# tachitachi/SR-WaveNet

Measured on NVIDIA B200. Metric: audio samples/sec, higher is better.
Workload: dtype f16

## Files before the change

sr-wavenet_b200/csrc/fused.cu:

```cuda
#include "common.cuh"
#include "mol.cuh"
#include "umma.cuh"
#include "philox.cuh"
#include <cuda_fp16.h>
#include <algorithm>
#include <cstdlib>

namespace fused {

constexpr int kTile = 128;
__host__ __device__ constexpr int tiles_of(bool teacher) { return teacher ? 3 : 4; }
__host__ __device__ constexpr int chunk_of(bool teacher) { return kTile * tiles_of(teacher); }
constexpr int kHalo = 512;
constexpr int kMaxLayers = 40;
constexpr int kMaxSeg = 8;

constexpr int kWfBytes = 64 * 32 * 2;
constexpr int kWrsTeacher = 32 * 160 * 2;
constexpr int kWrsStudent = 32 * 32 * 2;
constexpr int kH1Bytes = 128 * 128 * 2;
constexpr int kH2Bytes = 128 * 32 * 2;

struct Seg { int b, t_start, t_out, t_end; };

struct Params {
  const uint8_t* packed;
  const float* x_in;
  const float* x_scored;
  const float* cb;
  uint8_t* rings;
  const Seg* segs;
  const int* nseg;
  uint32_t* flags;
  int G;
  long long wait_limit;
  NoiseSpec noise;
  float* logits_out;
  float* nll_out;
  double* nll_partial;
  float* scale_out;
  float* mean_out;
  float* x_out;
  int* err;
#ifdef SRWN_TUNING
  long long* trace;
  int trace_chunk;
#endif
  int T, L, P, frames, O, M;
  int ring_bytes_per_team;
  int dil[kMaxLayers];
  int ring_off[kMaxLayers];
  int rsuf[kMaxLayers + 1];
};

template <bool TEACHER>
struct SmemMapT {
  static constexpr int NT = tiles_of(TEACHER);
  static constexpr int rows = kHalo + NT * kTile;
  static constexpr int hbuf = 0;
  static constexpr int hbuf_bytes = 4 * rows * 16;
  static constexpr int cbuf = hbuf + 2 * hbuf_bytes;
  static constexpr int cbuf_bytes = 4 * kTile * 16;
  static constexpr int wst = cbuf + NT * cbuf_bytes;
  static constexpr int wst_bytes = kWfBytes + (TEACHER ? kWrsTeacher : kWrsStudent);
  static constexpr int head = wst + 2 * wst_bytes;
  static constexpr int bias = head + (TEACHER ? kH1Bytes + kH2Bytes : 0);
  static constexpr int hbias = bias + kMaxLayers * 32 * 4;
  static constexpr int front = hbias + (128 + 128 + 32 + 64 + 4) * 4;
  static constexpr int cbs = front + 64 * 4;
  static constexpr int bars = cbs + NT * (kMaxLayers + 1) * 32 * 4;
  static constexpr int n_bars = 40;
  static constexpr int misc = bars + n_bars * 8;
  static constexpr int total = misc + 64;
};
static_assert(SmemMapT<true>::total <= 232448 && SmemMapT<false>::total <= 232448, "shared memory budget");
static_assert(3 * 16 * kTile * 16 <= 2 * SmemMapT<true>::hbuf_bytes, "head operand overlay");

template <int NT>
struct BarT {
  static constexpr int D1 = 0;
  static constexpr int D2 = NT;
  static constexpr int HD = 2 * NT;
  static constexpr int WFULL = 4 * NT;
  static constexpr int WEMPTY = WFULL + 2;
  static constexpr int HALO = WFULL + 4;
  static constexpr int G1 = WFULL + 6;
  static constexpr int HDD = WFULL + 8;
  static constexpr int TAIL = HDD + NT;
  static constexpr int C2 = TAIL + 1;
  static constexpr int count = C2 + 2 * NT;
};
static_assert(BarT<3>::count <= 40 && BarT<4>::count <= 40, "barrier slots");

using namespace umma;

__device__ __forceinline__ uint32_t gate2(f2_t a) {
  float a0, a1;
  upk(a, a0, a1);
  const f2_t f = pk(tanh_fast(a0), tanh_fast(a1));
  const f2_t s = mul2(f, f);
  f2_t t = fma2(s, pk(0.0017294071149080992f, 0.0017294071149080992f), pk(-0.020638039335608482f, -0.020638039335608482f));
  t = fma2(s, t, pk(0.2499687224626541f, 0.2499687224626541f));
  const f2_t c = fma2(f, pk(0.5f, 0.5f), mul2(s, t));
  float c0, c1;
  upk(c, c0, c1);
  return pack2(c0, c1);
}

__device__ __forceinline__ void store_row(uint8_t* buf, int rows_per_kc, int row, const float* v) {
#pragma unroll
  for (int kc = 0; kc < 4; kc++) {
    uint4 q;
    q.x = pack2(v[kc * 8 + 0], v[kc * 8 + 1]); q.y = pack2(v[kc * 8 + 2], v[kc * 8 + 3]);
    q.z = pack2(v[kc * 8 + 4], v[kc * 8 + 5]); q.w = pack2(v[kc * 8 + 6], v[kc * 8 + 7]);
    *reinterpret_cast<uint4*>(buf + ((size_t)kc * rows_per_kc + row) * 16) = q;
  }
}
__device__ __forceinline__ void store_row_packed(uint8_t* buf, int rows_per_kc, int row, const uint32_t* w) {
#pragma unroll
  for (int kc = 0; kc < 4; kc++)
    *reinterpret_cast<uint4*>(buf + ((size_t)kc * rows_per_kc + row) * 16) =
        make_uint4(w[kc * 4 + 0], w[kc * 4 + 1], w[kc * 4 + 2], w[kc * 4 + 3]);
}

#ifndef SRWN_TUNING
#define TRACE(role, layer, slot) do {} while (0)
#else
#define TRACE(role, layer, slot)                                                            \
  do {                                                                                      \
    if (tracing) p.trace[((role) * kMaxLayers + (layer)) * 12 + (slot)] = clock64();      \
  } while (0)
#endif

constexpr int kLoadWarp = 0;
__host__ __device__ constexpr int threads_of(bool handoff, int nt) { return (1 + 4 * nt + (handoff ? 1 : 0)) * 32; }

__device__ __noinline__ bool flag_spin(const uint32_t* f, uint32_t need, volatile int* abort_flag, const int* gerr, int code, long long limit) {
  const long long t0 = clock64();
  int spins = 0;
  uint32_t v;
  while (true) {
    __nanosleep(32);
    asm volatile("ld.acquire.gpu.global.u32 %0, [%1];" : "=r"(v) : "l"(f) : "memory");
    if (v >= need) return true;
    if (*abort_flag) return false;
    if (((++spins) & 1023) == 0 && *reinterpret_cast<const volatile int*>(gerr)) return false;
    if (clock64() - t0 > limit) {
      if (atomicCAS((int*)abort_flag, 0, 1) == 0) ((int*)abort_flag)[1] = code;
      return false;
    }
  }
}
__device__ __forceinline__ bool flag_try(const uint32_t* f, uint32_t need) {
  uint32_t v;
  asm volatile("ld.acquire.gpu.global.u32 %0, [%1];" : "=r"(v) : "l"(f) : "memory");
  if (v < need) return false;
  asm volatile("fence.proxy.async;" ::: "memory");
  return true;
}
__device__ __forceinline__ bool flag_wait(const uint32_t* f, uint32_t need, volatile int* abort_flag, const int* gerr, int code, long long limit) {
  uint32_t v;
  asm volatile("ld.acquire.gpu.global.u32 %0, [%1];" : "=r"(v) : "l"(f) : "memory");
  if (v < need && !flag_spin(f, need, abort_flag, gerr, code, limit)) return false;
  asm volatile("fence.proxy.async;" ::: "memory");
  return true;
}
__device__ __forceinline__ void ring_rows_done(uint32_t counter_addr, uint32_t rows) {
  asm volatile("red.release.cta.shared::cta.add.u32 [%0], %1;" ::"r"(counter_addr), "r"(rows) : "memory");
}
__device__ __forceinline__ int ring_rows_of(int d, int m, int chunk) {
  const int lo = max(chunk - d, m * kTile), hi = (m + 1) * kTile;
  return hi > lo ? hi - lo : 0;
}
__device__ __forceinline__ uint32_t ld_acquire_cta_shared(uint32_t addr) {
  uint32_t v;
  asm volatile("ld.acquire.cta.shared::cta.u32 %0, [%1];" : "=r"(v) : "r"(addr) : "memory");
  return v;
}
__device__ __forceinline__ void flag_publish(uint32_t* f, uint32_t chunks) {
  asm volatile("red.release.gpu.global.max.u32 [%0], %1;" ::"l"(f), "r"(chunks) : "memory");
}

template <bool TEACHER, bool HANDOFF>
__global__ void __launch_bounds__(threads_of(HANDOFF, tiles_of(TEACHER)), 1) k_fused(const Params p) {
  constexpr int NT = tiles_of(TEACHER), CH = NT * kTile;
  constexpr int kThreads = threads_of(HANDOFF, NT);
  constexpr int kPubWarp = 1 + 4 * NT;
  constexpr int TCOLS = TEACHER ? 160 : 64;
  using SM = SmemMapT<TEACHER>;
  constexpr int ROWS = SM::rows;
  using BR = BarT<NT>;
  constexpr int BAR_D1 = BR::D1, BAR_D2 = BR::D2, BAR_HD = BR::HD, BAR_WFULL = BR::WFULL, BAR_WEMPTY = BR::WEMPTY, BAR_HALO = BR::HALO,
                BAR_G1 = BR::G1, BAR_HDD = BR::HDD, BAR_TAIL = BR::TAIL, BAR_C2 = BR::C2;
  (void)BAR_HDD; (void)BAR_C2; (void)kPubWarp;
  extern __shared__ __align__(1024) uint8_t smem[];
  const int tid = threadIdx.x, lane = tid & 31, warp = tid >> 5;
  const uint32_t sbase = smem_u32(smem);
  volatile int* abort_flag = reinterpret_cast<volatile int*>(smem + SM::misc + 8);
  uint32_t* tmem_slot = reinterpret_cast<uint32_t*>(smem + SM::misc);
  auto bar = [&](int i) { return sbase + SM::bars + i * 8; };
  const int L = p.L;
  constexpr int wrs_bytes = TEACHER ? kWrsTeacher : kWrsStudent;
  constexpr int layer_bytes = kWfBytes + wrs_bytes;
  constexpr int wrs_rows = TEACHER ? 160 : 32;

  if (tid == 0) {
    for (int i = 0; i < NT; i++) {
      mbar_init(bar(BAR_D1 + i), 1); mbar_init(bar(BAR_D2 + i), 1); mbar_init(bar(BAR_HDD + i), 1);
      mbar_init(bar(BAR_C2 + 2 * i), 1); mbar_init(bar(BAR_C2 + 2 * i + 1), 1);
      mbar_init(bar(BAR_HD + 2 * i), kTile); mbar_init(bar(BAR_HD + 2 * i + 1), kTile);
    }
    for (int i = 0; i < 2; i++) {
      mbar_init(bar(BAR_WFULL + i), 1); mbar_init(bar(BAR_WEMPTY + i), NT);
      mbar_init(bar(BAR_HALO + i), 1); mbar_init(bar(BAR_G1 + i), NT);
    }
    mbar_init(bar(BAR_TAIL), 1);
    abort_flag[0] = 0; abort_flag[1] = 0;
    for (int i = 0; i < NT; i++) reinterpret_cast<volatile uint32_t*>(smem + SM::misc + 16)[i] = 0;
    asm volatile("fence.mbarrier_init.release.cluster;" ::: "memory");
  }
  {
    const uint8_t* pk_ = p.packed;
    const size_t off_fixed = (size_t)L * layer_bytes;
    const float* fbias = reinterpret_cast<const float*>(pk_ + off_fixed);
    float* s_bias = reinterpret_cast<float*>(smem + SM::bias);
    for (int i = tid; i < L * 32; i += kThreads) s_bias[i] = fbias[i];
    const float* ffront = fbias + kMaxLayers * 32;
    float* s_front = reinterpret_cast<float*>(smem + SM::front);
    for (int i = tid; i < 64; i += kThreads) s_front[i] = ffront[i];
    const float* fhb = ffront + 64;
    float* s_hb = reinterpret_cast<float*>(smem + SM::hbias);
    for (int i = tid; i < 128 + 128 + 32 + 64 + 4; i += kThreads) s_hb[i] = fhb[i];
    if (TEACHER) {
      const uint4* src = reinterpret_cast<const uint4*>(reinterpret_cast<const uint8_t*>(fhb + 128 + 128 + 32 + 64 + 4));
      uint4* dst = reinterpret_cast<uint4*>(smem + SM::head);
      for (int i = tid; i < (kH1Bytes + kH2Bytes) / 16; i += kThreads) dst[i] = src[i];
    }
  }
  fence_async_smem();
  if (warp == kLoadWarp) {
    asm volatile("tcgen05.alloc.cta_group::1.sync.aligned.shared::cta.b32 [%0], %1;" ::"r"(smem_u32(tmem_slot)), "r"(512));
    asm volatile("tcgen05.relinquish_alloc_permit.cta_group::1.sync.aligned;" ::);
  }
  tc_fence_before();
  __syncthreads();
  tc_fence_after();
  const uint32_t tmem = *tmem_slot;

  const int G = p.G, team = (int)blockIdx.x / G, member = (int)blockIdx.x % G;
  const Seg* segs = p.segs + (size_t)team * kMaxSeg;
  const int nseg = p.nseg[team];
  uint8_t* ring = p.rings + (size_t)team * p.ring_bytes_per_team;
  uint32_t* flags = p.flags + (size_t)team * kMaxLayers;
  const uint32_t ringcnt = sbase + SM::misc + 16;
  uint32_t pub_expect = 0;
  int seq = 0;
  int u0e = 0, u0o = 0, lay_base = 0;
  int chunk_idx = 0;
  int head_idx = 0;
  int tail_idx = 0;
  double nll_acc = 0.0;
  const bool elected = elect_one();

  for (int si = 0; si < nseg; si++) {
    const Seg sg = segs[si];
    for (int t0 = sg.t_start; t0 < sg.t_end; t0 += CH) {
      const int n = seq++;
      if (n % G != member) continue;
      const bool warm = TEACHER ? (t0 + CH <= sg.t_out) : false;
      const bool do_head = TEACHER && !warm;
      int Lc = L;
      if (t0 + CH <= sg.t_out) {
        const int dist = sg.t_out - (t0 + CH);
        Lc = 0;
        while (Lc < L && p.rsuf[Lc + 1] > dist) Lc++;
        if (Lc < 1) Lc = 1;
      }
#define U0(par) ((par) ? u0o : u0e)
#ifdef SRWN_TUNING
      const bool tracing_chunk = p.trace != nullptr && blockIdx.x == 0 && chunk_idx == p.trace_chunk;
#else
      constexpr bool tracing_chunk = false; (void)tracing_chunk;
#endif

      if (warp == kLoadWarp) {
        bool have_next = false;
        for (int l = 0; l < Lc; l++) {
          const int s = l & 1;
          const int use = U0(s) + (l >> 1);
          [[maybe_unused]] const bool tracing = tracing_chunk && lane == 0;
          TRACE(6, l, 0);
          if (l >= 2 && !mbar_wait(bar(BAR_G1 + s), (use - 1) & 1, abort_flag, 0x1100000 | l, p.wait_limit)) break;
          TRACE(6, l, 2);
          if (HANDOFF && n > 0 && !have_next &&
              !flag_wait(flags + l, (uint32_t)n, abort_flag, p.err, 0x1200000 | l, p.wait_limit)) break;
          have_next = false;
          const int d = p.dil[l];
          const uint8_t* rl = ring + p.ring_off[l];
          const uint32_t dst0 = sbase + SM::hbuf + s * SM::hbuf_bytes;
          const int slot0 = (int)((unsigned)t0 % (unsigned)d);
          if (t0 - d >= sg.t_start) {
            if (lane == 0) {
              mbar_expect_tx(bar(BAR_HALO + s), (uint32_t)(4 * d * 16));
              const uint32_t n1 = (uint32_t)(d - slot0) * 16, n2 = (uint32_t)slot0 * 16;
#pragma unroll
              for (int kc = 0; kc < 4; kc++) {
                const uint32_t dst = dst0 + (uint32_t)(kc * ROWS + kHalo - d) * 16;
                const uint8_t* src = rl + (size_t)kc * d * 16;
                asm volatile("cp.async.bulk.shared::cluster.global.mbarrier::complete_tx::bytes [%0], [%1], %2, [%3];"
                             ::"r"(dst), "l"(src + (size_t)slot0 * 16), "r"(n1), "r"(bar(BAR_HALO + s)) : "memory");
                if (n2)
                  asm volatile("cp.async.bulk.shared::cluster.global.mbarrier::complete_tx::bytes [%0], [%1], %2, [%3];"
                               ::"r"(dst + n1), "l"(src), "r"(n2), "r"(bar(BAR_HALO + s)) : "memory");
              }
            }
            __syncwarp();
          } else {
            for (int kc = 0; kc < 4; kc++) {
              for (int i = lane; i < d; i += 32) {
                const uint32_t dst = dst0 + (uint32_t)(kc * ROWS + kHalo - d + i) * 16;
                if (t0 - d + i >= sg.t_start) {
                  int slot = slot0 + i; if (slot >= d) slot -= d;
                  asm volatile("cp.async.cg.shared.global [%0], [%1], 16;" ::"r"(dst), "l"(rl + ((size_t)kc * d + slot) * 16) : "memory");
                } else {
                  asm volatile("st.shared.v4.u32 [%0], {%1, %1, %1, %1};" ::"r"(dst), "r"(0) : "memory");
                }
              }
            }
            asm volatile("cp.async.wait_all;" ::: "memory");
            fence_async_smem();
            __syncwarp();
            if (lane == 0) mbar_arrive(bar(BAR_HALO + s));
          }
          if (HANDOFF && n > 0 && l + 1 < Lc) have_next = flag_try(flags + l + 1, (uint32_t)n);
          if (!mbar_wait(bar(BAR_WEMPTY + s), (use & 1) ^ 1, abort_flag, 0x1000000 | l, p.wait_limit)) break;
          if (lane == 0) {
            mbar_expect_tx(bar(BAR_WFULL + s), layer_bytes);
            asm volatile("cp.async.bulk.shared::cluster.global.mbarrier::complete_tx::bytes [%0], [%1], %2, [%3];"
                         ::"r"(sbase + SM::wst + s * SM::wst_bytes),
                           "l"(p.packed + (size_t)l * layer_bytes), "r"(layer_bytes), "r"(bar(BAR_WFULL + s)) : "memory");
          }
          TRACE(6, l, 1);
          TRACE(6, l, 3);
        }
        if (Lc < L && !*abort_flag) {
          const bool ok = n == 0 || !HANDOFF || flag_wait(flags + Lc, (uint32_t)n, abort_flag, p.err, 0x1300000 | Lc, p.wait_limit);
          if (ok && lane == 0) mbar_arrive(bar(BAR_TAIL));
        }
      } else if (HANDOFF && warp == kPubWarp) {
        const int last = Lc < L - 1 ? Lc : L - 1;
        bool ok = true;
        for (int r = 0; r <= last && ok; r++) {
          if (lane < NT) {
            const int rows = ring_rows_of(p.dil[r], lane, CH);
            if (rows) {
              pub_expect += (uint32_t)rows;
              if ((int32_t)(ld_acquire_cta_shared(ringcnt + 4 * lane) - pub_expect) < 0) {
                const long long t0 = clock64();
                while ((int32_t)(ld_acquire_cta_shared(ringcnt + 4 * lane) - pub_expect) < 0) {
                  __nanosleep(128);
                  if (*abort_flag) { ok = false; break; }
                  if (clock64() - t0 > p.wait_limit) {
                    if (atomicCAS((int*)abort_flag, 0, 1) == 0) ((int*)abort_flag)[1] = 0x4000000 | (lane << 8) | r;
                    ok = false; break;
                  }
                }
              }
            }
          }
          ok = __all_sync(0xffffffffu, ok);
          if (ok && lane == 0) flag_publish(flags + r, (uint32_t)n + 1);
        }
        if (ok && lane == 0)
          for (int r = last + 1; r < L; r++) flag_publish(flags + r, (uint32_t)n + 1);
      } else {
        const int gw = warp & 3, m = (((warp - 1) >> 2) + gw + 1) % NT;
        const bool issuer = gw == m;
        const bool leader = issuer && elected;
        const int row = gw * 32 + lane;
        const uint32_t lane_addr = (uint32_t)(gw * 32) << 16;
        const int t = t0 + m * kTile + row;
        const bool in_utt = t < p.T;
        int frame = (t0 + m * kTile) / p.P;
        if (frame > p.frames - 1) frame = p.frames - 1;
        const float* cb_g = p.cb + ((size_t)sg.b * p.frames + frame) * (size_t)(L + 1) * 32;
        float* cb = reinterpret_cast<float*>(smem + SM::cbs) + m * (kMaxLayers + 1) * 32;
        for (int i = row; i < (L + 1) * 32; i += kTile) cb[i] = __ldg(cb_g + i);
        group_sync(m);
        const float* s_bias = reinterpret_cast<const float*>(smem + SM::bias);
        const float* s_front = reinterpret_cast<const float*>(smem + SM::front);
        const int rc = m * kTile + row;
        f2_t h2[16];
        float v[32];
        uint32_t w16[16];
        bool alive = true;
        [[maybe_unused]] const bool tracing = tracing_chunk && row == 0;
        constexpr uint32_t id32 = make_idesc(0, 128, 32), id128 = make_idesc(0, 128, 128);
        const uint32_t hb_lo0 = ((sbase + SM::hbuf) >> 4) + (uint32_t)(kHalo + m * kTile) + ((uint32_t)ROWS << 16);
        const uint32_t wb_lo0 = (sbase + SM::wst) >> 4;
        const uint32_t d_conv = tmem + m * TCOLS, d_skip = tmem + m * TCOLS + 32;
        uint32_t d_cop = d_skip;
        constexpr bool kLateG1 = !TEACHER && !HANDOFF;
        constexpr bool kLateWempty = !TEACHER && HANDOFF;

        {
          auto x_at = [&](int tt) -> float {
            const size_t i = (size_t)sg.b * p.T + tt;
            if (!TEACHER && p.noise.on) return philox::logistic_at(p.noise.seed, p.noise.stream, (uint64_t)i);
            return __ldg(p.x_in + i);
          };
          const float xm1 = (t >= 1 && t - 1 < p.T) ? x_at(t - 1) : 0.f;
          const float xm2 = (t >= 2 && t - 2 < p.T) ? x_at(t - 2) : 0.f;
#pragma unroll
          for (int j = 0; j < 16; j++) {
            const float a = fmaf(xm2, s_front[2 * j], fmaf(xm1, s_front[32 + 2 * j], cb[2 * j]));
            const float b = fmaf(xm2, s_front[2 * j + 1], fmaf(xm1, s_front[32 + 2 * j + 1], cb[2 * j + 1]));
            h2[j] = pk(a, b);
            w16[j] = pack2(a, b);
          }
          alive = mbar_wait(bar(BAR_HALO + 0), U0(0) & 1, abort_flag, 0x2000000 | (m << 8), p.wait_limit);
          store_row_packed(smem + SM::hbuf, ROWS, kHalo + rc, w16);
          const int d0 = p.dil[0];
          fence_async_smem();
          mbar_arrive(bar(BAR_HD + 2 * m + 0));
          if (rc >= CH - d0) store_row_packed(ring + p.ring_off[0], d0, t % d0, w16);
        }

        for (int l = 0; l < Lc; l++) {
          const int s = l & 1, sn = s ^ 1;
          const uint32_t ph = (lay_base + l) & 1, phs = (U0(s) + (l >> 1)) & 1;
          TRACE(m, l, 0);
          const uint32_t hb_lo = hb_lo0 + (uint32_t)(s * (SM::hbuf_bytes >> 4));
          const uint32_t wb_lo = wb_lo0 + (uint32_t)(s * (SM::wst_bytes >> 4));
          const uint32_t dl = (uint32_t)p.dil[l];
          const uint32_t b1_lo = wb_lo + (32u << 16);
          const uint32_t b2_lo = wb_lo + (kWfBytes >> 4) + ((uint32_t)wrs_rows << 16);
          if (gw == ((m + 3) & 3)) {
            alive = mbar_wait(bar(BAR_WFULL + s), phs, abort_flag, 0x3000000 | (m << 8) | l, p.wait_limit) && alive;
            if (NT > 3 && m >= 3) alive = mbar_wait(bar(BAR_HD + 2 * (m - 3) + s), phs, abort_flag, 0x3300000 | (m << 8) | l, p.wait_limit) && alive;
          }
          if (gw == ((m + 1) & 3) && m >= 1) alive = mbar_wait(bar(BAR_HD + 2 * (m - 1) + s), phs, abort_flag, 0x3100000 | (m << 8) | l, p.wait_limit) && alive;
          if (gw == ((m + 2) & 3) && m >= 2) alive = mbar_wait(bar(BAR_HD + 2 * (m - 2) + s), phs, abort_flag, 0x3200000 | (m << 8) | l, p.wait_limit) && alive;
          group_sync(m);
          TRACE(m, l, 1);
          if (HANDOFF && gw == (m == 0 ? 1 : 0) && lane == 0) {
            const int rows = ring_rows_of((int)dl, m, CH);
            if (rows) ring_rows_done(ringcnt + 4 * m, (uint32_t)rows);
          }
          if (issuer) {
            tc_fence_after();
            if (leader) {
              tc_mma<0>(d_conv, desc_from_lo(hb_lo - dl), desc_from_lo(b1_lo), id32);
              tc_mma<1>(d_conv, desc_from_lo(hb_lo - dl + 2 * ROWS), desc_from_lo(b1_lo + 64), id32);
              tc_mma<1>(d_conv, desc_from_lo(hb_lo), desc_from_lo(b1_lo + 128), id32);
              tc_mma<1>(d_conv, desc_from_lo(hb_lo + 2 * ROWS), desc_from_lo(b1_lo + 192), id32);
              tc_commit(bar(BAR_D1 + m));
              if constexpr (!kLateG1) tc_commit(bar(BAR_G1 + s));
            }
            __syncwarp();
          }
          TRACE(m, l, 2);
          bool next_ok = true;
          if (l + 1 < Lc && !issuer) {
            if (l >= 1) next_ok = mbar_poll(bar(BAR_G1 + sn), (U0(sn) + ((l - 1) >> 1)) & 1);
            next_ok = mbar_poll(bar(BAR_HALO + sn), (U0(sn) + ((l + 1) >> 1)) & 1) && next_ok;
          }

          alive = mbar_wait(bar(BAR_D1 + m), ph, abort_flag, 0x2100000 | (m << 8) | l, p.wait_limit) && alive;
          if (kLateG1 && gw == ((m + 2) & 3) && lane == 0) mbar_arrive(bar(BAR_G1 + s));
          TRACE(m, l, 3);
          tc_fence_after();
          tc_ld32(d_conv + lane_addr, v);
          tc_wait_ld();
          TRACE(m, l, 4);
          {
            const ulonglong2* b2 = reinterpret_cast<const ulonglong2*>(s_bias + l * 32);
#pragma unroll
            for (int q = 0; q < 8; q++) {
              const ulonglong2 bb = b2[q];
              const f2_t d0 = pk(v[4 * q], v[4 * q + 1]), d1 = pk(v[4 * q + 2], v[4 * q + 3]);
              w16[2 * q] = gate2(add2(d0, bb.x));
              w16[2 * q + 1] = gate2(add2(d1, bb.y));
            }
          }
          if constexpr (TEACHER) {
            const int cuse = lay_base + l, prev = m == 2 ? cuse : cuse - 1;
            d_cop = tmem + 480 + 16 * ((cuse + m) & 1);
            if (prev >= 0) alive = mbar_wait(bar(BAR_C2 + 2 * ((m + 1) % 3) + (prev & 1)), (uint32_t)((prev >> 1) & 1), abort_flag, 0x2800000 | (m << 8) | l, p.wait_limit) && alive;
            tc_fence_after();
          }
          tc_st16(d_cop + lane_addr, w16);
          tc_wait_st();
          tc_fence_before();
          TRACE(m, l, 5);
// ... 28 lines not shown
#pragma unroll
            for (int q = 0; q < 8; q++) {
              const ulonglong2 cc = c2[q];
              h2[2 * q] = fma2(add2(h2[2 * q], pk(v[4 * q], v[4 * q + 1])), sq, cc.x);
              h2[2 * q + 1] = fma2(add2(h2[2 * q + 1], pk(v[4 * q + 2], v[4 * q + 3])), sq, cc.y);
            }
          }
          TRACE(m, l, 9);
          if (l + 1 < L) {
#pragma unroll
            for (int j = 0; j < 16; j++) { float a, b; upk(h2[j], a, b); w16[j] = pack2(a, b); }
            if (l + 1 < Lc) {
              if (!next_ok) {
                if (l >= 1) alive = mbar_wait(bar(BAR_G1 + sn), (U0(sn) + ((l - 1) >> 1)) & 1, abort_flag, 0x2300000 | (m << 8) | l, p.wait_limit) && alive;
                alive = mbar_wait(bar(BAR_HALO + sn), (U0(sn) + ((l + 1) >> 1)) & 1, abort_flag, 0x2400000 | (m << 8) | l, p.wait_limit) && alive;
              }
              TRACE(m, l, 10);
              store_row_packed(smem + SM::hbuf + sn * SM::hbuf_bytes, ROWS, kHalo + rc, w16);
              tc_fence_before();
              fence_async_smem();
              mbar_arrive(bar(BAR_HD + 2 * m + sn));
            } else {
              tc_fence_before();
              alive = mbar_wait(bar(BAR_TAIL), tail_idx & 1, abort_flag, 0x2700000 | (m << 8) | l, p.wait_limit) && alive;
            }
            const int dn = p.dil[l + 1];
            if (rc >= CH - dn) store_row_packed(ring + p.ring_off[l + 1], dn, t % dn, w16);
            TRACE(m, l, 11);
          } else {
            tc_fence_before();
          }
        }

        if (TEACHER) {
          if (do_head) {
            const float* s_hb = reinterpret_cast<const float*>(smem + SM::hbias);
            uint8_t* a3 = smem + SM::hbuf + m * (16 * kTile * 16);
            const uint32_t a3_lo = ((sbase + SM::hbuf + m * (16 * kTile * 16)) >> 4) + ((uint32_t)kTile << 16);
            alive = mbar_wait(bar(BAR_G1 + ((L - 1) & 1)), (U0((L - 1) & 1) + ((L - 1) >> 1)) & 1, abort_flag, 0x2500000 | (m << 8), p.wait_limit) && alive;
            alive = mbar_wait(bar(BAR_WEMPTY + ((L - 1) & 1)), (U0((L - 1) & 1) + ((L - 1) >> 1)) & 1, abort_flag, 0x2510000 | (m << 8), p.wait_limit) && alive;
            tc_fence_after();
#pragma unroll 1
            for (int hs = 0; hs < 2; hs++) {
              for (int q = 0; q < 4; q++) {
                tc_ld32(d_skip + lane_addr + q * 32, v);
                tc_wait_ld();
#pragma unroll
                for (int j = 0; j < 32; j++) v[j] = fmaxf(v[j] + s_hb[hs * 128 + q * 32 + j], 0.f);
                store_row(a3 + (size_t)q * 4 * kTile * 16, kTile, row, v);
              }
              tc_fence_before();
              fence_async_smem();
              group_sync(m);
              if (issuer) {
                tc_fence_after();
                if (leader && !*abort_flag) {
                  const uint32_t wlo = ((sbase + SM::head + (hs == 0 ? 0 : kH1Bytes)) >> 4) + ((uint32_t)(hs == 0 ? 128 : 32) << 16);
                  const int nrows = hs == 0 ? 128 : 32;
#pragma unroll
                  for (int j = 0; j < 8; j++)
                    tc_mma_dyn(hs == 0 ? d_skip : d_conv, desc_from_lo(a3_lo + 2 * j * kTile), desc_from_lo(wlo + 2 * j * nrows),
                               hs == 0 ? id128 : id32, j);
                  tc_commit(bar(BAR_HDD + m));
                }
                __syncwarp();
              }
              alive = mbar_wait(bar(BAR_HDD + m), (head_idx * 2 + hs) & 1, abort_flag, 0x2600000 | (m << 8) | hs, p.wait_limit) && alive;
              tc_fence_after();
            }
            tc_ld32(d_conv + lane_addr, v);
            tc_wait_ld();
            tc_fence_before();
            if (alive && in_utt && t >= sg.t_out) {
#pragma unroll
              for (int j = 0; j < 32; j++) v[j] += s_hb[256 + j];
              const size_t at = (size_t)sg.b * p.T + t;
              float nl = 0.f;
              if (p.x_scored) {
                const float xs = __ldg(p.x_scored + at);
                if (p.M == 5) nl = mol_nll_fixed<5>(xs, v);
                else {
                  float lg[32];
#pragma unroll
                  for (int j = 0; j < 32; j++) lg[j] = v[j];
                  nl = mol_nll_one(xs, lg, p.M);
                }
              }
              if (p.logits_out) {
                float* dst = p.logits_out + at * p.O;
                if (p.O == 20) {
#pragma unroll
                  for (int j = 0; j < 5; j++)
                    reinterpret_cast<float4*>(dst)[j] = make_float4(v[4 * j], v[4 * j + 1], v[4 * j + 2], v[4 * j + 3]);
                } else {
#pragma unroll
                  for (int j = 0; j < 32; j++) if (j < p.O) dst[j] = v[j];
                }
              }
              if (p.x_scored) {
                if (p.nll_out) p.nll_out[at] = nl;
                nll_acc += (double)nl;
              }
            }
          }
        } else {
          const float* s_hb = reinterpret_cast<const float*>(smem + SM::hbias);
          const float* hk = s_hb + 288;
          float p0 = 0.f, p1 = 0.f;
#pragma unroll
          for (int j = 0; j < 16; j++) {
            float a, b;
            upk(h2[j], a, b);
            const float e0 = fmaxf(a, 0.f), e1 = fmaxf(b, 0.f);
            p0 = fmaf(e0, hk[4 * j], p0); p1 = fmaf(e0, hk[4 * j + 1], p1);
            p0 = fmaf(e1, hk[4 * j + 2], p0); p1 = fmaf(e1, hk[4 * j + 3], p1);
          }
          if (alive && in_utt && t >= sg.t_out) {
            const size_t at = (size_t)sg.b * p.T + t;
            const float sc = expf(p0 + hk[64]);
            const float mu = p1 + hk[65];
            p.scale_out[at] = sc;
            p.mean_out[at] = mu;
            const float xin = p.noise.on ? philox::logistic_at(p.noise.seed, p.noise.stream, (uint64_t)at) : __ldg(p.x_in + at);
            p.x_out[at] = fmaf(xin, sc, mu);
          }
        }
      }
      if (HANDOFF && Lc < L && warp != kLoadWarp && warp != kPubWarp) {
        const int gw = warp & 3, m = (((warp - 1) >> 2) + gw + 1) % NT;
        group_sync(m);
        if (gw == (m == 0 ? 1 : 0) && lane == 0) {
          const int rows = ring_rows_of(p.dil[Lc], m, CH);
          if (rows) ring_rows_done(ringcnt + 4 * m, (uint32_t)rows);
        }
      }
      if (do_head) head_idx++;
      if (Lc < L) tail_idx++;
      chunk_idx++;
      u0e += (Lc + 1) >> 1; u0o += Lc >> 1; lay_base += Lc;
      tc_fence_before();
      asm volatile("fence.proxy.async;" ::: "memory");
      __syncthreads();
      tc_fence_after();
      if (*abort_flag) break;
    }
    if (*abort_flag) break;
  }

  if (TEACHER && p.nll_partial) {
    double* s_red = reinterpret_cast<double*>(smem + SM::cbuf);
    for (int s = 16; s >= 1; s >>= 1) nll_acc += __shfl_xor_sync(0xffffffffu, nll_acc, s);
    if (lane == 0) s_red[warp] = nll_acc;
    __syncthreads();
    if (tid == 0) {
      double tot = 0;
      for (int w = 1; w <= 4 * NT; w++) tot += s_red[w];
      p.nll_partial[blockIdx.x] = tot;
    }
  }
  if (tid == 0 && *abort_flag) {
    volatile int* e = p.err;
    e[1] = abort_flag[1]; e[2] = chunk_idx; e[3] = blockIdx.x;
    __threadfence_system();
    e[0] = 1;
  }
  tc_fence_before();
  __syncthreads();
  if (warp == kLoadWarp) {
    tc_fence_after();
    asm volatile("tcgen05.dealloc.cta_group::1.sync.aligned.b32 %0, %1;" ::"r"(tmem), "r"(512));
  }
}

__global__ void k_sum_partials(const double* __restrict__ part, int n, float* __restrict__ out) {
  double tot = 0;
  for (int i = threadIdx.x; i < n; i += 32) tot += part[i];
  for (int s = 16; s >= 1; s >>= 1) tot += __shfl_xor_sync(0xffffffffu, tot, s);
  if (threadIdx.x == 0) *out = (float)tot;
}

__global__ void k_fold_bias(const float* __restrict__ cond, const float* __restrict__ front_b,
                            const float* __restrict__ res_b, float* __restrict__ cb, int L) {
  const int bf = blockIdx.x;
  for (int o = threadIdx.x; o < (L + 1) * 32; o += blockDim.x) {
    const int i = o / 32, j = o % 32;
    float v = i < L ? cond[((size_t)bf * L + i) * 32 + j] : 0.f;
    v += i == 0 ? front_b[j] : SRWN_SQRT_HALF * res_b[(i - 1) * 32 + j];
    cb[(size_t)bf * (L + 1) * 32 + o] = v;
  }
}


// ... 220 lines not shown
    if (force_G > 0 && G != std::min(force_G, std::min(kMaxTeam, grid))) continue;
    int teams = grid / G;
    if ((long long)teams > total) teams = (int)total;
    if (teams < 1) continue;
    Partition cand = partition_for(B, T, kChunk, warm_cost, teams);
    const double lag = kLagLayers / L;
    const double period = std::max(1.0, G * lag);
    const double time = (cand.cost / G + (G > 1 ? 0.5 : 0.0)) * period * (G > 1 ? handoff_cost : 1.0) + (G - 1) * lag;
    if (time < best_time) { best_time = time; best = cand; best.G = G; }
  }
  return best;
}

struct FusedWs {
  float* cb; uint8_t* rings; uint32_t* flags; double* partial;
#ifdef SRWN_TUNING
  long long* trace;
#endif
  float *scales, *means, *xa, *xb;
  size_t bytes;
};

static FusedWs carve_fused(const srwn_ctx* c, int B, int T, void* ws, size_t cap) {
  WsCarver w(ws, cap);
  FusedWs r{};
  const size_t frames = T / c->cfg.pool_stride, L = c->cfg.n_layers, n = (size_t)B * T;
  const int grid = c->sm_count > 0 ? c->sm_count : 148;
  const size_t nst = c->cfg.kind == SRWN_STUDENT ? (size_t)c->cfg.num_flows : 1;
  r.cb = w.take<float>((size_t)B * frames * (L + 1) * 32 * nst);
  r.rings = w.take<uint8_t>((size_t)grid * ((size_t)c->sum_dilation * 64 + 256));
  r.flags = w.take<uint32_t>((size_t)grid * kMaxLayers * nst);
  r.partial = w.take<double>(grid);
#ifdef SRWN_TUNING
  r.trace = w.take<long long>(7 * kMaxLayers * 12);
#endif
  if (c->cfg.kind == SRWN_STUDENT) {
    r.scales = w.take<float>(n * c->cfg.num_flows);
    r.means = w.take<float>(n * c->cfg.num_flows);
    r.xa = w.take<float>(n);
    r.xb = w.take<float>(n);
  }
  r.bytes = w.used;
  return r;
}

size_t fused_partition_bytes(const srwn_ctx* c) {
  const size_t grid = c->sm_count > 0 ? c->sm_count : 148;
  return grid * kMaxSeg * sizeof(Seg) + grid * sizeof(int);
}

size_t fused_workspace_bytes(const srwn_ctx* c, int op, int B, int T) {
  return carve_fused(c, B, T, nullptr, 0).bytes;
}

template <bool TEACHER>
static int launch_fused(srwn_ctx* c, const Params& p, int grid, cudaStream_t st) {
  const bool handoff = p.G > 1;
  auto kern = handoff ? k_fused<TEACHER, true> : k_fused<TEACHER, false>;
  SRWN_CUDA(cudaFuncSetAttribute(kern, cudaFuncAttributeMaxDynamicSharedMemorySize, SmemMapT<TEACHER>::total));
  Params pl = p;
  void* args[] = {&pl};
  SRWN_CUDA(cudaLaunchCooperativeKernel((const void*)kern, dim3(grid), dim3(threads_of(handoff, tiles_of(TEACHER))), args, SmemMapT<TEACHER>::total, st));
  SRWN_LAUNCH_CHECK();
  return SRWN_OK;
}

static int sticky_error(const srwn_ctx* c) {
// ... 90 lines not shown
  for (int f = 0; f < F; f++) {
    Params p;
    int rc = prepare(c, f, enc, B, T, w, &p, &grid, f == 0, st);
    if (rc) return rc;
    float* xout = (f == F - 1 && x_last) ? x_last : ((f & 1) ? w.xb : w.xa);
    p.x_in = xin; p.scale_out = w.scales + (size_t)f * n; p.mean_out = w.means + (size_t)f * n; p.x_out = xout;
    if (f == 0) p.noise = noise;
    ProfScope prof(c, st, "k_fused<student,fp16>", 1);
    rc = launch_fused<false>(c, p, grid, st);
    if (rc) return rc;
    xin = xout;
  }
  return run_flow_compose(z, noise, z_out, w.scales, w.means, F, out, s_tot, mu_tot, (int64_t)n, st);
}

int fused_check_error(void* ws, size_t ws_bytes, const srwn_ctx* c, int B, int T, cudaStream_t st) {
  (void)ws; (void)ws_bytes; (void)B; (void)T;
  SRWN_CUDA(cudaStreamSynchronize(st));
  volatile int* e = c->h_err;
  if (e && e[0]) {
    const int code = e[1], chunk = e[2], cta = e[3];
    e[0] = 0; e[1] = 0; e[2] = 0; e[3] = 0;
    return srwn_fail(SRWN_ERR_CUDA, "fused kernel aborted: pipeline wait timed out (code 0x%x, chunk %d, cta %d)", code, chunk, cta);
  }
  return SRWN_OK;
}

void fused_last_partition(const srwn_ctx* c, int* teams, int* G) { *teams = c->part_teams; *G = c->part_G; }

#ifdef SRWN_TUNING
extern "C" int srwn_debug_read_trace(srwn_handle_t h, int32_t B, int32_t T, void* ws, size_t ws_bytes,
                                     long long* out, int32_t count) {
  FusedWs w = carve_fused(h, B, T, ws, ws_bytes);
  if (count > 7 * kMaxLayers * 12) count = 7 * kMaxLayers * 12;
  SRWN_CUDA(cudaDeviceSynchronize());
  SRWN_CUDA(cudaMemcpy(out, w.trace, sizeof(long long) * count, cudaMemcpyDeviceToHost));
  return SRWN_OK;
}

namespace fused {
template <int N, int CNT>
__device__ __forceinline__ void bench_issue(uint32_t tmem_col, uint32_t a_lo, uint32_t b_lo, uint32_t mbar_addr) {
  constexpr uint32_t idesc = make_idesc(0, 128, N);
#pragma unroll
  for (int i = 0; i < CNT; i++) {
    if (i == 0) tc_mma<0>(tmem_col, desc_from_lo(a_lo), desc_from_lo(b_lo), idesc);
    else tc_mma<1>(tmem_col, desc_from_lo(a_lo + (i & 3) * 256), desc_from_lo(b_lo + (i & 3) * 64), idesc);
  }
  tc_commit(mbar_addr);
}

__global__ void __launch_bounds__(416, 1) k_mma_bench(long long* out) {
  extern __shared__ __align__(1024) uint8_t smem[];
  __shared__ uint32_t tmem_slot;
  __shared__ __align__(8) uint64_t mbar[16];
  __shared__ long long s_t[16][2];
  const uint32_t sbase = smem_u32(smem);
  const int warp = threadIdx.x >> 5;
  for (int i = threadIdx.x; i < 65536 / 4; i += 416) reinterpret_cast<uint32_t*>(smem)[i] = 0x3c003c00u;
  if (threadIdx.x == 0) {
    for (int i = 0; i < 16; i++) mbar_init(smem_u32(&mbar[i]), 1);
    asm volatile("fence.mbarrier_init.release.cluster;" ::: "memory");
  }
  fence_async_smem();
  if (warp == 0) {
    asm volatile("tcgen05.alloc.cta_group::1.sync.aligned.shared::cta.b32 [%0], %1;" ::"r"(smem_u32(&tmem_slot)), "r"(512));
    asm volatile("tcgen05.relinquish_alloc_permit.cta_group::1.sync.aligned;" ::);
// ... 61 lines not shown
```

Before: 910.1 million.

## Prefetch next chunk's weights, conditioning, input and halo during current chunk tail

In the teacher non-handoff kernel, the load warp now finds the next chunk assigned to the CTA and, once the current chunk's layers are issued, starts bulk async copies of its first two layers' weights, its conditioning bias rows, its input samples and its layer-0 halo. Compute warps no longer load conditioning with __ldg and read neighbouring x values from shared memory, guarded by new CB/CBFREE mbarriers. The aim is to hide the load latency at chunk boundaries and head processing. In exchange there is more barrier bookkeeping and phase-parity logic that could deadlock or race, plus extra tuning-only trace stamps.

```diff
diff --git a/sr-wavenet_b200/csrc/fused.cu b/sr-wavenet_b200/csrc/fused.cu
--- a/sr-wavenet_b200/csrc/fused.cu
+++ b/sr-wavenet_b200/csrc/fused.cu
@@ -22,6 +22,13 @@
 constexpr int kH2Bytes = 128 * 32 * 2;
 
 struct Seg { int b, t_start, t_out, t_end; };
+
+#ifdef SRWN_TUNING
+constexpr int kTraceStamps = 7 * kMaxLayers * 12;
+constexpr int kTraceChunks = 128;
+constexpr int kTraceLongs = kTraceStamps + 4 * (kTraceChunks + 1);
+constexpr int kBoundRow = kMaxLayers - 1;
+#endif
 
 struct Params {
   const uint8_t* packed;
@@ -88,7 +95,9 @@
   static constexpr int HDD = WFULL + 8;
   static constexpr int TAIL = HDD + NT;
   static constexpr int C2 = TAIL + 1;
-  static constexpr int count = C2 + 2 * NT;
+  static constexpr int CB = C2 + 2 * NT;
+  static constexpr int CBFREE = CB + 1;
+  static constexpr int count = CBFREE + 1;
 };
 static_assert(BarT<3>::count <= 40 && BarT<4>::count <= 40, "barrier slots");
 
@@ -125,10 +134,17 @@
 
 #ifndef SRWN_TUNING
 #define TRACE(role, layer, slot) do {} while (0)
+#define TRACE_IF(cond, role, layer, slot) do {} while (0)
+#define TRACE_REC(cond, i) do {} while (0)
 #else
-#define TRACE(role, layer, slot)                                                            \
+#define TRACE_IF(cond, role, layer, slot)                                                   \
   do {                                                                                      \
-    if (tracing) p.trace[((role) * kMaxLayers + (layer)) * 12 + (slot)] = clock64();      \
+    if (cond) p.trace[((role) * kMaxLayers + (layer)) * 12 + (slot)] = clock64();         \
+  } while (0)
+#define TRACE(role, layer, slot) TRACE_IF(tracing, role, layer, slot)
+#define TRACE_REC(cond, i)                                                                  \
+  do {                                                                                      \
+    if (cond) p.trace[kTraceStamps + (i)] = clock64();                                     \
   } while (0)
 #endif
 
@@ -181,6 +197,28 @@
   asm volatile("red.release.gpu.global.max.u32 [%0], %1;" ::"l"(f), "r"(chunks) : "memory");
 }
 
+__device__ __forceinline__ int chunk_layers(const Params& p, int L, const Seg& sg, int t0, int CH) {
+  int Lc = L;
+  if (t0 + CH <= sg.t_out) {
+    const int dist = sg.t_out - (t0 + CH);
+    Lc = 0;
+    while (Lc < L && p.rsuf[Lc + 1] > dist) Lc++;
+    if (Lc < 1) Lc = 1;
+  }
+  return Lc;
+}
+__device__ __forceinline__ bool next_chunk(const Seg* segs, int nseg, int si, int t0, int seq, int G, int member, int CH,
+                                           int& si_n, int& t0_n) {
+  int t = t0 + CH;
+  for (int i = si; i < nseg; i++) {
+    const Seg sg = segs[i];
+    if (i > si) t = sg.t_start;
+    for (; t < sg.t_end; t += CH, seq++)
+      if (seq % G == member) { si_n = i; t0_n = t; return true; }
+  }
+  return false;
+}
+
 template <bool TEACHER, bool HANDOFF>
 __global__ void __launch_bounds__(threads_of(HANDOFF, tiles_of(TEACHER)), 1) k_fused(const Params p) {
   constexpr int NT = tiles_of(TEACHER), CH = NT * kTile;
@@ -191,8 +229,9 @@
   constexpr int ROWS = SM::rows;
   using BR = BarT<NT>;
   constexpr int BAR_D1 = BR::D1, BAR_D2 = BR::D2, BAR_HD = BR::HD, BAR_WFULL = BR::WFULL, BAR_WEMPTY = BR::WEMPTY, BAR_HALO = BR::HALO,
-                BAR_G1 = BR::G1, BAR_HDD = BR::HDD, BAR_TAIL = BR::TAIL, BAR_C2 = BR::C2;
+                BAR_G1 = BR::G1, BAR_HDD = BR::HDD, BAR_TAIL = BR::TAIL, BAR_C2 = BR::C2, BAR_CB = BR::CB, BAR_CBFREE = BR::CBFREE;
   (void)BAR_HDD; (void)BAR_C2; (void)kPubWarp;
+  constexpr bool kStageAhead = TEACHER && !HANDOFF;
   extern __shared__ __align__(1024) uint8_t smem[];
   const int tid = threadIdx.x, lane = tid & 31, warp = tid >> 5;
   const uint32_t sbase = smem_u32(smem);
@@ -215,6 +254,7 @@
       mbar_init(bar(BAR_HALO + i), 1); mbar_init(bar(BAR_G1 + i), NT);
     }
     mbar_init(bar(BAR_TAIL), 1);
+    if (kStageAhead) { mbar_init(bar(BAR_CB), 1); mbar_init(bar(BAR_CBFREE), 4 * NT); }
     abort_flag[0] = 0; abort_flag[1] = 0;
     for (int i = 0; i < NT; i++) reinterpret_cast<volatile uint32_t*>(smem + SM::misc + 16)[i] = 0;
     asm volatile("fence.mbarrier_init.release.cluster;" ::: "memory");
@@ -261,6 +301,71 @@
   int tail_idx = 0;
   double nll_acc = 0.0;
   const bool elected = elect_one();
+#ifdef SRWN_TUNING
+  const bool trace_cta = p.trace != nullptr && blockIdx.x == 0;
+#else
+  constexpr bool trace_cta = false; (void)trace_cta;
+#endif
+  TRACE_REC(trace_cta && tid == 0, 4 * kTraceChunks);
+  auto issue_weights = [&](int l, int s) {
+    mbar_expect_tx(bar(BAR_WFULL + s), layer_bytes);
+    asm volatile("cp.async.bulk.shared::cluster.global.mbarrier::complete_tx::bytes [%0], [%1], %2, [%3];"
+                 ::"r"(sbase + SM::wst + s * SM::wst_bytes),
+                   "l"(p.packed + (size_t)l * layer_bytes), "r"(layer_bytes), "r"(bar(BAR_WFULL + s)) : "memory");
+  };
+  auto issue_halo_bulk = [&](int l, int s, int t0x) {
+    const int d = p.dil[l];
+    const uint8_t* rl = ring + p.ring_off[l];
+    const uint32_t dst0 = sbase + SM::hbuf + s * SM::hbuf_bytes;
+    const int slot0 = (int)((unsigned)t0x % (unsigned)d);
+    mbar_expect_tx(bar(BAR_HALO + s), (uint32_t)(4 * d * 16));
+    const uint32_t n1 = (uint32_t)(d - slot0) * 16, n2 = (uint32_t)slot0 * 16;
+#pragma unroll
+    for (int kc = 0; kc < 4; kc++) {
+      const uint32_t dst = dst0 + (uint32_t)(kc * ROWS + kHalo - d) * 16;
+      const uint8_t* src = rl + (size_t)kc * d * 16;
+      asm volatile("cp.async.bulk.shared::cluster.global.mbarrier::complete_tx::bytes [%0], [%1], %2, [%3];"
+                   ::"r"(dst), "l"(src + (size_t)slot0 * 16), "r"(n1), "r"(bar(BAR_HALO + s)) : "memory");
+      if (n2)
+        asm volatile("cp.async.bulk.shared::cluster.global.mbarrier::complete_tx::bytes [%0], [%1], %2, [%3];"
+                     ::"r"(dst + n1), "l"(src), "r"(n2), "r"(bar(BAR_HALO + s)) : "memory");
+    }
+  };
+  const bool x_staged = kStageAhead && (reinterpret_cast<uintptr_t>(p.x_in) & 15) == 0;
+  auto stage_chunk = [&](const Seg& sgx, int t0x, int Lcx, int u0e_x, int u0o_x, int cbfree_par) -> bool {
+    for (int l = 0; l < 2 && l < Lcx; l++) {
+      if (!mbar_wait(bar(BAR_WEMPTY + l), ((l ? u0o_x : u0e_x) & 1) ^ 1, abort_flag, 0x1000000 | l, p.wait_limit)) return false;
+      if (lane == 0) issue_weights(l, l);
+    }
+    if (cbfree_par >= 0 && !mbar_wait(bar(BAR_CBFREE), (uint32_t)cbfree_par, abort_flag, 0x1400000, p.wait_limit)) return false;
+    if (lane == 0) {
+      const uint32_t bytes = (uint32_t)(L + 1) * 32 * 4;
+      const int xb = t0x >= 4 ? t0x - 4 : 0, xe = min(p.T, t0x + CH);
+      const uint32_t xbytes = x_staged ? (uint32_t)(xe - xb) * 4 : 0u;
+      mbar_expect_tx(bar(BAR_CB), NT * bytes + xbytes);
+      if (xbytes)
+        asm volatile("cp.async.bulk.shared::cluster.global.mbarrier::complete_tx::bytes [%0], [%1], %2, [%3];"
+                     ::"r"(sbase + SM::cbuf), "l"(p.x_in + (size_t)sgx.b * p.T + xb), "r"(xbytes), "r"(bar(BAR_CB)) : "memory");
+#pragma unroll 1
+      for (int m = 0; m < NT; m++) {
+        int frame = (t0x + m * kTile) / p.P;
+        if (frame > p.frames - 1) frame = p.frames - 1;
+        asm volatile("cp.async.bulk.shared::cluster.global.mbarrier::complete_tx::bytes [%0], [%1], %2, [%3];"
+                     ::"r"(sbase + SM::cbs + (uint32_t)(m * (kMaxLayers + 1) * 32 * 4)),
+                       "l"(p.cb + ((size_t)sgx.b * p.frames + frame) * (size_t)(L + 1) * 32), "r"(bytes), "r"(bar(BAR_CB)) : "memory");
+      }
+    }
+    __syncwarp();
+    return true;
+  };
+  auto stage_halo0 = [&](int Lcx) -> bool {
+    const int sl = (Lcx - 1) & 1;
+    if (!mbar_wait(bar(BAR_G1 + sl), ((sl ? u0o : u0e) + ((Lcx - 1) >> 1)) & 1, abort_flag, 0x1500000, p.wait_limit)) return false;
+    asm volatile("fence.proxy.async;" ::: "memory");
+    return true;
+  };
+  bool staged = false;
+  bool halo0_staged = false;
 
   for (int si = 0; si < nseg; si++) {
     const Seg sg = segs[si];
@@ -269,23 +374,23 @@
       if (n % G != member) continue;
       const bool warm = TEACHER ? (t0 + CH <= sg.t_out) : false;
       const bool do_head = TEACHER && !warm;
-      int Lc = L;
-      if (t0 + CH <= sg.t_out) {
-        const int dist = sg.t_out - (t0 + CH);
-        Lc = 0;
-        while (Lc < L && p.rsuf[Lc + 1] > dist) Lc++;
-        if (Lc < 1) Lc = 1;
-      }
+      const int Lc = chunk_layers(p, L, sg, t0, CH);
 #define U0(par) ((par) ? u0o : u0e)
 #ifdef SRWN_TUNING
-      const bool tracing_chunk = p.trace != nullptr && blockIdx.x == 0 && chunk_idx == p.trace_chunk;
+      const bool tracing_chunk = trace_cta && chunk_idx == p.trace_chunk;
+      const bool tracing_next = trace_cta && chunk_idx == p.trace_chunk + 1;
+      const bool rec_chunk = trace_cta && chunk_idx < kTraceChunks;
+      if (rec_chunk && tid == 0) p.trace[kTraceStamps + 4 * chunk_idx] = Lc + (do_head ? 100 : 0);
 #else
-      constexpr bool tracing_chunk = false; (void)tracing_chunk;
+      constexpr bool tracing_chunk = false, tracing_next = false, rec_chunk = false;
+      (void)tracing_chunk; (void)tracing_next; (void)rec_chunk;
 #endif
 
       if (warp == kLoadWarp) {
         bool have_next = false;
-        for (int l = 0; l < Lc; l++) {
+        TRACE_IF(tracing_next && lane == 0, 6, kBoundRow, 0);
+        const bool started = !kStageAhead || staged || stage_chunk(sg, t0, Lc, u0e, u0o, -1);
+        for (int l = 0; started && l < Lc; l++) {
           const int s = l & 1;
           const int use = U0(s) + (l >> 1);
           [[maybe_unused]] const bool tracing = tracing_chunk && lane == 0;
@@ -299,21 +404,9 @@
           const uint8_t* rl = ring + p.ring_off[l];
           const uint32_t dst0 = sbase + SM::hbuf + s * SM::hbuf_bytes;
           const int slot0 = (int)((unsigned)t0 % (unsigned)d);
-          if (t0 - d >= sg.t_start) {
-            if (lane == 0) {
-              mbar_expect_tx(bar(BAR_HALO + s), (uint32_t)(4 * d * 16));
-              const uint32_t n1 = (uint32_t)(d - slot0) * 16, n2 = (uint32_t)slot0 * 16;
-#pragma unroll
-              for (int kc = 0; kc < 4; kc++) {
-                const uint32_t dst = dst0 + (uint32_t)(kc * ROWS + kHalo - d) * 16;
-                const uint8_t* src = rl + (size_t)kc * d * 16;
-                asm volatile("cp.async.bulk.shared::cluster.global.mbarrier::complete_tx::bytes [%0], [%1], %2, [%3];"
-                             ::"r"(dst), "l"(src + (size_t)slot0 * 16), "r"(n1), "r"(bar(BAR_HALO + s)) : "memory");
-                if (n2)
-                  asm volatile("cp.async.bulk.shared::cluster.global.mbarrier::complete_tx::bytes [%0], [%1], %2, [%3];"
-                               ::"r"(dst + n1), "l"(src), "r"(n2), "r"(bar(BAR_HALO + s)) : "memory");
-              }
-            }
+          if (kStageAhead && l == 0 && halo0_staged) {
+          } else if (t0 - d >= sg.t_start) {
+            if (lane == 0) issue_halo_bulk(l, s, t0);
             __syncwarp();
           } else {
             for (int kc = 0; kc < 4; kc++) {
@@ -332,21 +425,33 @@
             __syncwarp();
             if (lane == 0) mbar_arrive(bar(BAR_HALO + s));
           }
+          TRACE_IF(tracing_next && lane == 0 && l == 0, 6, kBoundRow, 1);
           if (HANDOFF && n > 0 && l + 1 < Lc) have_next = flag_try(flags + l + 1, (uint32_t)n);
-          if (!mbar_wait(bar(BAR_WEMPTY + s), (use & 1) ^ 1, abort_flag, 0x1000000 | l, p.wait_limit)) break;
-          if (lane == 0) {
-            mbar_expect_tx(bar(BAR_WFULL + s), layer_bytes);
-            asm volatile("cp.async.bulk.shared::cluster.global.mbarrier::complete_tx::bytes [%0], [%1], %2, [%3];"
-                         ::"r"(sbase + SM::wst + s * SM::wst_bytes),
-                           "l"(p.packed + (size_t)l * layer_bytes), "r"(layer_bytes), "r"(bar(BAR_WFULL + s)) : "memory");
+          if (!kStageAhead || l >= 2) {
+            if (!mbar_wait(bar(BAR_WEMPTY + s), (use & 1) ^ 1, abort_flag, 0x1000000 | l, p.wait_limit)) break;
+            if (lane == 0) issue_weights(l, s);
           }
           TRACE(6, l, 1);
           TRACE(6, l, 3);
         }
+        TRACE_IF(tracing_chunk && lane == 0, 6, kBoundRow, 3);
         if (Lc < L && !*abort_flag) {
           const bool ok = n == 0 || !HANDOFF || flag_wait(flags + Lc, (uint32_t)n, abort_flag, p.err, 0x1300000 | Lc, p.wait_limit);
           if (ok && lane == 0) mbar_arrive(bar(BAR_TAIL));
         }
+        staged = false;
+        halo0_staged = false;
+        int si_n, t0_n;
+        if (kStageAhead && !*abort_flag && next_chunk(segs, nseg, si, t0, seq, G, member, CH, si_n, t0_n)) {
+          const Seg sgn = segs[si_n];
+          staged = stage_chunk(sgn, t0_n, chunk_layers(p, L, sgn, t0_n, CH), u0e + ((Lc + 1) >> 1), u0o + (Lc >> 1), chunk_idx & 1);
+          if (staged && t0_n - p.dil[0] >= sgn.t_start && stage_halo0(Lc)) {
+            if (lane == 0) issue_halo_bulk(0, 0, t0_n);
+            __syncwarp();
+            halo0_staged = true;
+          }
+        }
+        TRACE_IF(tracing_chunk && lane == 0, 6, kBoundRow, 2);
       } else if (HANDOFF && warp == kPubWarp) {
         const int last = Lc < L - 1 ? Lc : L - 1;
         bool ok = true;
@@ -381,12 +486,14 @@
         const uint32_t lane_addr = (uint32_t)(gw * 32) << 16;
         const int t = t0 + m * kTile + row;
         const bool in_utt = t < p.T;
-        int frame = (t0 + m * kTile) / p.P;
-        if (frame > p.frames - 1) frame = p.frames - 1;
-        const float* cb_g = p.cb + ((size_t)sg.b * p.frames + frame) * (size_t)(L + 1) * 32;
         float* cb = reinterpret_cast<float*>(smem + SM::cbs) + m * (kMaxLayers + 1) * 32;
-        for (int i = row; i < (L + 1) * 32; i += kTile) cb[i] = __ldg(cb_g + i);
-        group_sync(m);
+        if constexpr (!kStageAhead) {
+          int frame = (t0 + m * kTile) / p.P;
+          if (frame > p.frames - 1) frame = p.frames - 1;
+          const float* cb_g = p.cb + ((size_t)sg.b * p.frames + frame) * (size_t)(L + 1) * 32;
+          for (int i = row; i < (L + 1) * 32; i += kTile) cb[i] = __ldg(cb_g + i);
+          group_sync(m);
+        }
         const float* s_bias = reinterpret_cast<const float*>(smem + SM::bias);
         const float* s_front = reinterpret_cast<const float*>(smem + SM::front);
         const int rc = m * kTile + row;
@@ -409,8 +516,19 @@
             if (!TEACHER && p.noise.on) return philox::logistic_at(p.noise.seed, p.noise.stream, (uint64_t)i);
             return __ldg(p.x_in + i);
           };
-          const float xm1 = (t >= 1 && t - 1 < p.T) ? x_at(t - 1) : 0.f;
-          const float xm2 = (t >= 2 && t - 2 < p.T) ? x_at(t - 2) : 0.f;
+          float xm1, xm2;
+          if (x_staged) {
+            alive = mbar_wait(bar(BAR_CB), chunk_idx & 1, abort_flag, 0x2900000 | (m << 8), p.wait_limit) && alive;
+            const float* xs = reinterpret_cast<const float*>(smem + SM::cbuf);
+            const int xb = t0 >= 4 ? t0 - 4 : 0;
+            xm1 = (t >= 1 && t - 1 < p.T) ? xs[t - 1 - xb] : 0.f;
+            xm2 = (t >= 2 && t - 2 < p.T) ? xs[t - 2 - xb] : 0.f;
+          } else {
+            xm1 = (t >= 1 && t - 1 < p.T) ? x_at(t - 1) : 0.f;
+            xm2 = (t >= 2 && t - 2 < p.T) ? x_at(t - 2) : 0.f;
+            if (kStageAhead) alive = mbar_wait(bar(BAR_CB), chunk_idx & 1, abort_flag, 0x2900000 | (m << 8), p.wait_limit) && alive;
+          }
+          TRACE_IF(tracing_next && row == 0, m, kBoundRow, 9);
 #pragma unroll
           for (int j = 0; j < 16; j++) {
             const float a = fmaf(xm2, s_front[2 * j], fmaf(xm1, s_front[32 + 2 * j], cb[2 * j]));
@@ -418,11 +536,13 @@
             h2[j] = pk(a, b);
             w16[j] = pack2(a, b);
           }
+          TRACE_IF(tracing_next && row == 0, m, kBoundRow, 10);
           alive = mbar_wait(bar(BAR_HALO + 0), U0(0) & 1, abort_flag, 0x2000000 | (m << 8), p.wait_limit);
           store_row_packed(smem + SM::hbuf, ROWS, kHalo + rc, w16);
           const int d0 = p.dil[0];
           fence_async_smem();
           mbar_arrive(bar(BAR_HD + 2 * m + 0));
+          TRACE_IF(tracing_next && row == 0, m, kBoundRow, 11);
           if (rc >= CH - d0) store_row_packed(ring + p.ring_off[0], d0, t % d0, w16);
         }
 
@@ -437,12 +557,15 @@
           const uint32_t b2_lo = wb_lo + (kWfBytes >> 4) + ((uint32_t)wrs_rows << 16);
           if (gw == ((m + 3) & 3)) {
             alive = mbar_wait(bar(BAR_WFULL + s), phs, abort_flag, 0x3000000 | (m << 8) | l, p.wait_limit) && alive;
+            TRACE_IF(tracing_next && l == 0 && lane == 0, m, kBoundRow - 1, 2);
             if (NT > 3 && m >= 3) alive = mbar_wait(bar(BAR_HD + 2 * (m - 3) + s), phs, abort_flag, 0x3300000 | (m << 8) | l, p.wait_limit) && alive;
           }
           if (gw == ((m + 1) & 3) && m >= 1) alive = mbar_wait(bar(BAR_HD + 2 * (m - 1) + s), phs, abort_flag, 0x3100000 | (m << 8) | l, p.wait_limit) && alive;
           if (gw == ((m + 2) & 3) && m >= 2) alive = mbar_wait(bar(BAR_HD + 2 * (m - 2) + s), phs, abort_flag, 0x3200000 | (m << 8) | l, p.wait_limit) && alive;
           group_sync(m);
           TRACE(m, l, 1);
+          TRACE_IF(tracing_next && l == 0 && row == 0, m, kBoundRow - 1, 0);
+          TRACE_REC(rec_chunk && l == 0 && m == 0 && row == 0, 4 * chunk_idx + 1);
           if (HANDOFF && gw == (m == 0 ? 1 : 0) && lane == 0) {
             const int rows = ring_rows_of((int)dl, m, CH);
             if (rows) ring_rows_done(ringcnt + 4 * m, (uint32_t)rows);
@@ -460,6 +583,7 @@
             __syncwarp();
           }
           TRACE(m, l, 2);
+          TRACE_IF(tracing_next && l == 0 && row == 0, m, kBoundRow - 1, 1);
           bool next_ok = true;
           if (l + 1 < Lc && !issuer) {
             if (l >= 1) next_ok = mbar_poll(bar(BAR_G1 + sn), (U0(sn) + ((l - 1) >> 1)) & 1);
@@ -554,6 +678,14 @@
           }
         }
 
+        auto cb_free = [&]() {
+          if constexpr (kStageAhead) {
+            __syncwarp();
+            if (lane == 0) mbar_arrive(bar(BAR_CBFREE));
+          }
+        };
+        if (!do_head) cb_free();
+        TRACE_REC(rec_chunk && m == 0 && row == 0, 4 * chunk_idx + 2);
         if (TEACHER) {
           if (do_head) {
             const float* s_hb = reinterpret_cast<const float*>(smem + SM::hbias);
@@ -574,6 +706,7 @@
               tc_fence_before();
               fence_async_smem();
               group_sync(m);
+              TRACE_IF(tracing, m, kBoundRow, 3 * hs);
               if (issuer) {
                 tc_fence_after();
                 if (leader && !*abort_flag) {
@@ -587,12 +720,16 @@
                 }
                 __syncwarp();
               }
+              TRACE_IF(tracing, m, kBoundRow, 3 * hs + 1);
               alive = mbar_wait(bar(BAR_HDD + m), (head_idx * 2 + hs) & 1, abort_flag, 0x2600000 | (m << 8) | hs, p.wait_limit) && alive;
+              TRACE_IF(tracing, m, kBoundRow, 3 * hs + 2);
               tc_fence_after();
             }
+            cb_free();
             tc_ld32(d_conv + lane_addr, v);
             tc_wait_ld();
             tc_fence_before();
+            TRACE_IF(tracing, m, kBoundRow, 6);
             if (alive && in_utt && t >= sg.t_out) {
 #pragma unroll
               for (int j = 0; j < 32; j++) v[j] += s_hb[256 + j];
@@ -624,6 +761,7 @@
                 nll_acc += (double)nl;
               }
             }
+            TRACE_IF(tracing, m, kBoundRow, 7);
           }
         } else {
           const float* s_hb = reinterpret_cast<const float*>(smem + SM::hbias);
@@ -664,6 +802,8 @@
       asm volatile("fence.proxy.async;" ::: "memory");
       __syncthreads();
       tc_fence_after();
+      TRACE_IF(tracing_chunk && tid == 0, 6, kBoundRow, 8);
+      TRACE_REC(rec_chunk && tid == 0, 4 * (chunk_idx - 1) + 3);
       if (*abort_flag) break;
     }
     if (*abort_flag) break;
@@ -680,6 +820,10 @@
       p.nll_partial[blockIdx.x] = tot;
     }
   }
+  TRACE_REC(trace_cta && tid == 0, 4 * kTraceChunks + 1);
+#ifdef SRWN_TUNING
+  if (trace_cta && tid == 0) p.trace[kTraceStamps + 4 * kTraceChunks + 2] = chunk_idx;
+#endif
   if (tid == 0 && *abort_flag) {
     volatile int* e = p.err;
     e[1] = abort_flag[1]; e[2] = chunk_idx; e[3] = blockIdx.x;
@@ -966,7 +1110,7 @@
   r.flags = w.take<uint32_t>((size_t)grid * kMaxLayers * nst);
   r.partial = w.take<double>(grid);
 #ifdef SRWN_TUNING
-  r.trace = w.take<long long>(7 * kMaxLayers * 12);
+  r.trace = w.take<long long>(kTraceLongs);
 #endif
   if (c->cfg.kind == SRWN_STUDENT) {
     r.scales = w.take<float>(n * c->cfg.num_flows);
@@ -1123,7 +1267,7 @@
 extern "C" int srwn_debug_read_trace(srwn_handle_t h, int32_t B, int32_t T, void* ws, size_t ws_bytes,
                                      long long* out, int32_t count) {
   FusedWs w = carve_fused(h, B, T, ws, ws_bytes);
-  if (count > 7 * kMaxLayers * 12) count = 7 * kMaxLayers * 12;
+  if (count > kTraceLongs) count = kTraceLongs;
   SRWN_CUDA(cudaDeviceSynchronize());
   SRWN_CUDA(cudaMemcpy(out, w.trace, sizeof(long long) * count, cudaMemcpyDeviceToHost));
   return SRWN_OK;
```

Measured after the change: 930.1 million, median of 6. +2.2%, better.
